# transferia/transferia

Measured on AMD Instinct MI355X. Metric: ChangeItems/sec through CSV parse -> mask(ClientIP)+filter(EventDate) -> devnull, ClickBench hits, HBM-resident input (the PCIe-inclusive rate is `pcie_inclusive`), higher is better.
Workload: dtype u8; 1 GPU; ClickBench hits-1M CSV parse -> mask(ip)+filter(EventDate) -> devnull (BASELINE.json configs[1]); columns=105, parallelism=row-range shard x1, no collective, rows_per_pass=1048576, csv_bytes_per_pass=838371857

## Files before the change

transferia_amd/csrc/tf_common.hpp:

```cpp
#pragma once
#include <hip/hip_runtime.h>

#include <cstdint>
#include <cstdio>
#include <cstring>
#include <memory>
#include <mutex>
#include <unordered_map>
#include <stdexcept>
#include <string>
#include <vector>

#include "../../include/tfgpu.h"

#ifndef TF_DYNAMIC_LDS
#define TF_DYNAMIC_LDS(type, name) extern __shared__ type name[]
#endif

#ifndef TF_GLOBAL_PTR
#define TF_GLOBAL_PTR(T, p) ((T *)(__attribute__((address_space(1))) T *)(p))
#endif

#ifndef TF_CONST_PTR
#define TF_CONST_PTR(T, p) ((const __attribute__((address_space(4))) T *)(p))
#endif

#ifndef TF_KEEP
#define TF_KEEP(x) asm volatile("" ::"v"(x))
#endif
#ifndef TF_OPAQUE
#define TF_OPAQUE(x) asm volatile("" : "+v"(x))
#endif

struct tfgpu_dbatch;

namespace tf {

struct Error : std::runtime_error {
  int code;
  Error(int c, const std::string &m) : std::runtime_error(m), code(c) {}
};
void set_last_error(const std::string &m);
int fail(int code, const std::string &m);

#define TF_HIP(expr)                                                                              \
  do {                                                                                            \
    hipError_t e__ = (expr);                                                                      \
    if (e__ != hipSuccess)                                                                        \
      throw ::tf::Error(TFGPU_ERR_DEVICE, std::string(#expr) + ": " + hipGetErrorString(e__));    \
  } while (0)

struct ProfEntry {
  std::string name;
  int64_t launches = 0;
  double total_ms = 0;
  int64_t units = 0;
};

struct BlockCache {
  std::mutex mu;
  std::unordered_map<size_t, std::vector<void *>> free_;
  size_t cached = 0;
  void *get(size_t cls);
  void put(void *p, size_t cls);
  void trim();
};

struct Context {
  int device = -1;
  hipStream_t stream = nullptr;
  hipStream_t copy_stream = nullptr;
  BlockCache blocks;
  void *pin_base = nullptr;
  size_t pin_cap = 0, pin_off = 0;
  void *pin(size_t bytes);
  template <class T> T *pin_n(size_t n) { return reinterpret_cast<T *>(pin(n * sizeof(T))); }
  bool prof_on = false;
  std::vector<ProfEntry> prof;
  struct Pending { int idx; hipEvent_t a, b; int64_t units = 0; };
  std::vector<Pending> pending;
  std::vector<hipEvent_t> free_events;
  hipEvent_t dense_event = nullptr;
  std::mutex mu;
  int num_cus = 256;
  std::shared_ptr<struct DevMem> pow10tab;
  struct ConstEntry { uint64_t hash; std::vector<uint8_t> bytes; std::shared_ptr<struct DevMem> mem; uint64_t stamp; };
  std::vector<ConstEntry> consts;
  uint64_t const_clock = 0;
  double csv_hint_bpl = 0.0;
  int csv_hint_ncols = -1;

  hipEvent_t get_event();
  void prof_begin(const char *name, Pending &p);
  void prof_end(Pending &p);
  void prof_flush();
};
Context &ctx();
int bind_lane(int lane);
int current_lane();
int lane_device(int lane);
struct LaneScope {
  int prev;
  explicit LaneScope(int lane) : prev(bind_lane(lane)) {}
// ... 37 lines not shown
void sync();

inline bool repr_is_var(int r) { return r == TFGPU_R_STRING || r == TFGPU_R_BYTES || r == TFGPU_R_JSONNUM || r == TFGPU_R_JSON; }
inline size_t repr_width(int r) {
  switch (r) {
    case TFGPU_R_INT8: case TFGPU_R_UINT8: case TFGPU_R_BOOL: return 1;
    case TFGPU_R_INT16: case TFGPU_R_UINT16: return 2;
    case TFGPU_R_INT32: case TFGPU_R_UINT32: case TFGPU_R_FLOAT32: return 4;
    case TFGPU_R_INT64: case TFGPU_R_UINT64: case TFGPU_R_FLOAT64: case TFGPU_R_TIME: case TFGPU_R_DURATION: return 8;
    default: return 0;
  }
}

struct TextView {
  Buf src;
  Buf fstart;
  uint8_t quote = '"';
  bool jsonnum = false;
  bool has_special = true;
  Buf packed;
};
struct DColumn {
  std::string name;
  int dtype = TFGPU_T_INVALID;
  int repr = TFGPU_R_INVALID;
  Buf values, offsets, data, nanos, validity;
  Buf absent;
  uint64_t data_len = 0;
  std::shared_ptr<TextView> view;
  const Buf &payload() const { return (!data && view) ? view->packed : data; }
  bool lazy() const { return !data && view && !view->packed; }
};
void materialize(const struct ::tfgpu_dbatch &b, const std::vector<const DColumn *> *only = nullptr);
void dense(const struct ::tfgpu_dbatch *b, bool absent_ok = false);
void dense_locked(const struct ::tfgpu_dbatch &b);
int lanes_created();
uint64_t lane_generation();
std::unique_ptr<struct ::tfgpu_dbatch> snapshot(const struct ::tfgpu_dbatch &b);
bool has_absent(const struct ::tfgpu_dbatch &b);
Buf validity_minus_absent(const Buf &validity, const Buf &absent, int64_t nrows);
Buf find_device_block(const void *p);
void register_device_block(const Buf &b);

}

namespace tf {
struct PendingRows {
  std::shared_ptr<const struct ::tfgpu_dbatch> src;
  Buf sel;
};
}

struct tfgpu_dbatch {
  int64_t nrows = 0;
  std::vector<tf::DColumn> cols;
  std::shared_ptr<tf::PendingRows> pending;
  void *dense_done = nullptr;
  int dense_lane = -1;
  uint64_t dense_gen = 0;
  std::vector<tf::DColumn> replaced;
  std::vector<std::pair<std::string, int>> schema;
  std::vector<std::string> key_names;
  std::vector<tf::DColumn> old_keys;
  tf::Buf old_present;
  std::string ns, table;
  tf::Buf kind, src_row, part_id;
  tf::Buf col_order;
};

struct tfgpu_dbuf {
  tf::Buf mem;
  uint64_t size = 0;
};

namespace tf {
inline std::unique_ptr<tfgpu_dbatch> shallow_copy(const tfgpu_dbatch &in) { return std::make_unique<tfgpu_dbatch>(in); }
template <class F> void materialize_where(const tfgpu_dbatch &b, F pred) {
  std::vector<const DColumn *> need;
  for (auto &c : b.cols) if (pred(c)) need.push_back(&c);
  materialize(b, &need);
}
void exclusive_scan_u32(const uint32_t *in, uint32_t *out, int64_t n, bool with_total);
void exclusive_scan_u32_segments(uint32_t *inout, int64_t seg_len, int nseg, int64_t seg_stride);
const uint32_t *any_nonzero_to_host(const uint32_t *v, int64_t n);
const uint32_t *segment_totals_to_host(const uint32_t *scanned, int64_t seg_len, int nseg, int64_t seg_stride);
void sum_u32_segments_u64(const uint32_t *in, int64_t seg_len, int nseg, int64_t seg_stride, unsigned long long *totals);

}
```

transferia_amd/csrc/tf_csv.hip:

```cpp
#include <algorithm>
#include <cmath>
#include <cstdio>
#include <type_traits>

#include "tf_devfmt.hpp"
#include "tf_devparse.hpp"
#include "tf_devfloat.hpp"
#include "tf_segcopy.hpp"
#include "tf_textview.hpp"
#include "tf_wave.hpp"
#include "tf_swar.hpp"
#include "tf_gotime.hpp"
#include "tf_f64range.hpp"
#include "tf_plan.hpp"
#include "tf_strictcell.hpp"

#ifdef TF_CSV_ABLATE_BUILD
#define CSV_ABL(x) ((x).ablate)
#else
#define CSV_ABL(x) 0
#endif
namespace tf {

std::unique_ptr<tfgpu_dbatch> compact_rows(const tfgpu_dbatch &in, Buf keep);

static constexpr int NL_THREADS = 256;
#ifndef TF_NL_ITERS
#define TF_NL_ITERS 7
#endif
static constexpr int NL_ITERS = TF_NL_ITERS;
static constexpr int NL_TILE = NL_THREADS * 16 * NL_ITERS;
static constexpr int CSV_GRAN = 64 * 16;
static constexpr int NL_GPT = NL_TILE / CSV_GRAN;
static_assert(NL_TILE == NL_GPT * CSV_GRAN && NL_THREADS * 16 == 4 * CSV_GRAN, "a wave iteration is a granule");

__device__ __forceinline__ uint32_t nl_mask16(uint4 v) {
  uint32_t m = 0;
  const uint32_t w[4] = {v.x, v.y, v.z, v.w};
#pragma unroll
  for (int k = 0; k < 4; k++) {
    uint32_t x = w[k] ^ 0x0A0A0A0Au;
    uint32_t b0 = ((x & 0xFFu) == 0), b1 = ((x & 0xFF00u) == 0), b2 = ((x & 0xFF0000u) == 0), b3 = ((x & 0xFF000000u) == 0);
    m |= (b0 | b1 << 1 | b2 << 2 | b3 << 3) << (4 * k);
  }
  return m;
}
__device__ __forceinline__ uint32_t nl_count16(uint4 v) {
  const uint32_t w[4] = {v.x, v.y, v.z, v.w};
  uint32_t acc = 0;
#pragma unroll
  for (int k = 0; k < 4; k++) {
    const uint32_t x = w[k] ^ 0x0A0A0A0Au;
    const uint32_t z = ~(((x & 0x7F7F7F7Fu) + 0x7F7F7F7Fu) | x) & 0x80808080u;
    acc = __builtin_amdgcn_udot4(z >> 7, 0x01010101u, acc, false);
  }
  return acc;
}

__device__ __forceinline__ uint4 load16_guard(const uint8_t *base, uint64_t pos, uint64_t len) {
  uint4 v = *reinterpret_cast<const uint4 *>(base + pos);
  if (pos + 16 > len) {
    uint32_t w[4] = {v.x, v.y, v.z, v.w};
    for (int i = 0; i < 16; i++) if (pos + i >= len) w[i >> 2] &= ~(0xFFu << (8 * (i & 3)));
    v = make_uint4(w[0], w[1], w[2], w[3]);
  }
  return v;
}

__global__ void __launch_bounds__(NL_THREADS) csv_count_newlines(const uint8_t *__restrict__ data, uint64_t len, uint32_t *__restrict__ gran_counts, int64_t ngran) {
  const uint64_t tile = (uint64_t)blockIdx.x * NL_TILE;
  const int lane = threadIdx.x & 63, wv = threadIdx.x >> 6;
#pragma unroll
  for (int it = 0; it < NL_ITERS; it++) {
    const uint64_t pos = tile + ((uint64_t)it * NL_THREADS + threadIdx.x) * 16;
    uint32_t cnt = 0;
    if (pos < len) cnt = nl_count16(load16_guard(data, pos, len));
    const uint32_t inc = wave_scan_add(cnt);
    const int64_t g = (int64_t)blockIdx.x * NL_GPT + it * 4 + wv;
    if (lane == 63 && g < ngran) gran_counts[g] = inc;
  }
}

__global__ void __launch_bounds__(NL_THREADS) csv_line_index(const uint8_t *__restrict__ data, uint64_t len, const uint32_t *__restrict__ tile_base,
                                                            uint32_t *__restrict__ row_start ) {
  __shared__ uint32_t wsum[NL_THREADS / 64];
  uint64_t tile = (uint64_t)blockIdx.x * NL_TILE;
  uint32_t base = tile_base[(int64_t)blockIdx.x * NL_GPT];
  const int lane = threadIdx.x & 63, wv = threadIdx.x >> 6;
  for (int it = 0; it < NL_ITERS; it++) {
    uint64_t pos = tile + ((uint64_t)it * NL_THREADS + threadIdx.x) * 16;
    uint32_t m = pos < len ? nl_mask16(load16_guard(data, pos, len)) : 0;
    uint32_t c = __popc(m), inc = c;
    for (int d = 1; d < 64; d <<= 1) { uint32_t t = __shfl_up(inc, d, 64); if (lane >= d) inc += t; }
    if (lane == 63) wsum[wv] = inc;
    __syncthreads();
    uint32_t wbase = 0, tot = 0;
    for (int i = 0; i < NL_THREADS / 64; i++) { uint32_t s = wsum[i]; if (i < wv) wbase += s; tot += s; }
    __syncthreads();
    uint32_t k = base + wbase + inc - c;
    while (m) { int b = __ffs(m) - 1; m &= m - 1; row_start[++k] = (uint32_t)(pos + b + 1); }
    base += tot;
  }
}


template <class F> __device__ __forceinline__ uint32_t space_prefix(const F &f, uint32_t i, uint32_t end) {
  uint32_t c = f[i];
  if (c == ' ' || (c >= 9 && c <= 13)) return 1;
  if (c < 0xC2) return 0;
  uint32_t r = end - i;
  if (c == 0xC2 && r >= 2) { uint32_t d = f[i + 1]; return (d == 0x85 || d == 0xA0) ? 2 : 0; }
  if (r >= 3 && (c == 0xE1 || c == 0xE2 || c == 0xE3)) {
    uint32_t d = f[i + 1], e = f[i + 2];
    if (c == 0xE1) return (d == 0x9A && e == 0x80) ? 3 : 0;
    if (c == 0xE3) return (d == 0x80 && e == 0x80) ? 3 : 0;
    if (d == 0x80 && ((e >= 0x80 && e <= 0x8A) || e == 0xA8 || e == 0xA9 || e == 0xAF)) return 3;
    if (d == 0x81 && e == 0x9F) return 3;
  }
  return 0;
}
template <class F> __device__ __forceinline__ uint32_t space_suffix(const F &f, uint32_t a, uint32_t b) {
  uint32_t c = f[b - 1];
  if (c == ' ' || (c >= 9 && c <= 13)) return 1;
  if (c < 0x80) return 0;
  if (b - a >= 2 && f[b - 2] == 0xC2 && (c == 0x85 || c == 0xA0)) return 2;
  if (b - a >= 3 && space_prefix(f, b - 3, b) == 3) return 3;
  return 0;
}

struct CsvOpts {
  uint8_t delim, quote, escape, double_quote, include_missing, strings_can_be_null, quoted_strings_can_be_null, pad;
  int32_t n_null, n_true, n_false;
  const uint32_t *list_off;
  const uint8_t *list_data;
  GtSet user_tp;
  GtSet cast_tp;
  const uint8_t *dp;
  uint32_t dp_len;
  uint32_t multiline;
  const uint64_t *p128;
};

__device__ __forceinline__ bool any_quote(const uint32_t *qmask, uint32_t lo, uint32_t hi) {
  if (lo >= hi) return false;
  const uint32_t w0 = lo >> 5, w1 = (hi - 1) >> 5;
  for (uint32_t w = w0; w <= w1; w++) {
    uint32_t m = qmask[w];
    if (w == w0) m &= ~0u << (lo & 31);
    if (w == w1) m &= ~0u >> (31 - ((hi - 1) & 31));
    if (m) return true;
  }
  return false;
}

// ... 2258 lines not shown
```

transferia_amd/csrc/tf_mask.hip:

```cpp
#include "tf_plan.hpp"
#include "tf_rows.hpp"
#include "tf_devrow.hpp"
#include "tf_emit.hpp"

namespace tf {
__constant__ uint32_t SHA_K[64] = {
    0x428a2f98, 0x71374491, 0xb5c0fbcf, 0xe9b5dba5, 0x3956c25b, 0x59f111f1, 0x923f82a4, 0xab1c5ed5, 0xd807aa98, 0x12835b01, 0x243185be,
    0x550c7dc3, 0x72be5d74, 0x80deb1fe, 0x9bdc06a7, 0xc19bf174, 0xe49b69c1, 0xefbe4786, 0x0fc19dc6, 0x240ca1cc, 0x2de92c6f, 0x4a7484aa,
    0x5cb0a9dc, 0x76f988da, 0x983e5152, 0xa831c66d, 0xb00327c8, 0xbf597fc7, 0xc6e00bf3, 0xd5a79147, 0x06ca6351, 0x14292967, 0x27b70a85,
    0x2e1b2138, 0x4d2c6dfc, 0x53380d13, 0x650a7354, 0x766a0abb, 0x81c2c92e, 0x92722c85, 0xa2bfe8a1, 0xa81a664b, 0xc24b8b70, 0xc76c51a3,
    0xd192e819, 0xd6990624, 0xf40e3585, 0x106aa070, 0x19a4c116, 0x1e376c08, 0x2748774c, 0x34b0bcb5, 0x391c0cb3, 0x4ed8aa4a, 0x5b9cca4f,
    0x682e6ff3, 0x748f82ee, 0x78a5636f, 0x84c87814, 0x8cc70208, 0x90befffa, 0xa4506ceb, 0xbef9a3f7, 0xc67178f2};

__device__ __forceinline__ uint32_t rotr32(uint32_t x, int n) { return __builtin_rotateright32(x, n); }

__device__ __forceinline__ void sha256_compress(uint32_t st[8], uint32_t w[16]) {
  uint32_t a = st[0], b = st[1], c = st[2], d = st[3], e = st[4], f = st[5], g = st[6], h = st[7];
#pragma unroll
  for (int i = 0; i < 64; i++) {
    if (i >= 16) {
      uint32_t w15 = w[(i - 15) & 15], w2 = w[(i - 2) & 15];
      uint32_t s0 = rotr32(w15, 7) ^ rotr32(w15, 18) ^ (w15 >> 3);
      uint32_t s1 = rotr32(w2, 17) ^ rotr32(w2, 19) ^ (w2 >> 10);
      w[i & 15] = w[i & 15] + s0 + w[(i - 7) & 15] + s1;
    }
    uint32_t t1 = h + (rotr32(e, 6) ^ rotr32(e, 11) ^ rotr32(e, 25)) + ((e & f) ^ (~e & g)) + SHA_K[i] + w[i & 15];
    uint32_t t2 = (rotr32(a, 2) ^ rotr32(a, 13) ^ rotr32(a, 22)) + ((a & b) ^ (a & c) ^ (b & c));
    h = g; g = f; f = e; e = d + t1; d = c; c = b; b = a; a = t1 + t2;
  }
  st[0] += a; st[1] += b; st[2] += c; st[3] += d; st[4] += e; st[5] += f; st[6] += g; st[7] += h;
}

struct MaskParams {
  DCol col;
  uint32_t ipad[8], opad[8];
  int64_t nrows;
  uint8_t *out;
  const int32_t *sel;
};

struct Text24 {
  uint64_t t0 = 0, t1 = 0, t2 = 0; uint32_t n = 0;
  __device__ __forceinline__ void put_word(uint64_t w, uint32_t k) {
    const uint32_t at = n & 7u, sh = at * 8, seg = n >> 3;
    const uint64_t lo = w << sh, hi = (w >> 1) >> (63 - sh);
    if (seg == 0) { t0 |= lo; t1 |= hi; } else if (seg == 1) { t1 |= lo; t2 |= hi; } else t2 |= lo;
    n += k;
  }
  __device__ __forceinline__ void put(uint32_t c) { put_word(c & 0xFFu, 1); }
};
__device__ __forceinline__ bool mask_small_int(const DCol &c, int64_t r, Text24 &s) {
  if (!is_valid(c, r)) { s.put_word(0x3E6C696E3Cull , 5); return true; }
  switch (c.repr) {
    case TFGPU_R_INT8: emit_i64(s, ((const int8_t *)c.values)[r]); return true;
    case TFGPU_R_INT16: emit_i64(s, ((const int16_t *)c.values)[r]); return true;
    case TFGPU_R_INT32: emit_i64(s, ((const int32_t *)c.values)[r]); return true;
    case TFGPU_R_INT64: emit_i64(s, ((const int64_t *)c.values)[r]); return true;
    case TFGPU_R_UINT8: emit_u64(s, ((const uint8_t *)c.values)[r]); return true;
    case TFGPU_R_UINT16: emit_u64(s, ((const uint16_t *)c.values)[r]); return true;
    case TFGPU_R_UINT32: emit_u64(s, ((const uint32_t *)c.values)[r]); return true;
    case TFGPU_R_UINT64: emit_u64(s, ((const uint64_t *)c.values)[r]); return true;
    default: return false;
  }
}

__global__ void __launch_bounds__(256) mask_hmac_kernel(MaskParams p) {
  const int64_t ro = (int64_t)blockIdx.x * blockDim.x + threadIdx.x;
  if (ro >= p.nrows) return;
  const int64_t r = p.sel ? (int64_t)p.sel[ro] : ro;
  uint32_t st[8], w[16];
#pragma unroll
  for (int i = 0; i < 8; i++) st[i] = p.ipad[i];
  const bool small_int = p.col.repr >= TFGPU_R_INT8 && p.col.repr <= TFGPU_R_UINT64;
  if (small_int) {
    Text24 s;
    mask_small_int(p.col, r, s);
    const uint32_t len = s.n;
    s.put_word(0x80, 1);
    w[0] = __builtin_bswap32((uint32_t)s.t0); w[1] = __builtin_bswap32((uint32_t)(s.t0 >> 32));
    w[2] = __builtin_bswap32((uint32_t)s.t1); w[3] = __builtin_bswap32((uint32_t)(s.t1 >> 32));
    w[4] = __builtin_bswap32((uint32_t)s.t2); w[5] = __builtin_bswap32((uint32_t)(s.t2 >> 32));
#pragma unroll
    for (int i = 6; i < 15; i++) w[i] = 0;
    w[15] = (64 + len) * 8;
    sha256_compress(st, w);
  } else {
  uint8_t buf[64];
  const uint8_t *ext;
  int len = serialize_small(p.col, r, buf, &ext);
  int off = 0;
  uint64_t bits = (uint64_t)(64 + len) * 8;
  bool pad_done = false, len_done = false;
  while (!len_done) {
#pragma unroll
    for (int i = 0; i < 16; i++) w[i] = 0;
    int take = len - off; if (take > 64) take = 64; if (take < 0) take = 0;
    for (int i = 0; i < take; i++) {
      uint32_t b = ext ? ext[off + i] : buf[off + i];
      w[i >> 2] |= b << (24 - 8 * (i & 3));
    }
    off += take;
    if (take < 64 && !pad_done) { w[take >> 2] |= 0x80u << (24 - 8 * (take & 3)); pad_done = true; if (take < 56) { w[14] = (uint32_t)(bits >> 32); w[15] = (uint32_t)bits; len_done = true; } }
    else if (pad_done) { w[14] = (uint32_t)(bits >> 32); w[15] = (uint32_t)bits; len_done = true; }
    sha256_compress(st, w);
  }
  }
#pragma unroll
  for (int i = 0; i < 8; i++) w[i] = st[i];
  w[8] = 0x80000000u;
#pragma unroll
  for (int i = 9; i < 15; i++) w[i] = 0;
  w[15] = (64 + 32) * 8;
  uint32_t so[8];
#pragma unroll
  for (int i = 0; i < 8; i++) so[i] = p.opad[i];
  sha256_compress(so, w);
  uint4 *dst = reinterpret_cast<uint4 *>(p.out + ro * 64);
#pragma unroll
  for (int q = 0; q < 4; q++) {
    uint32_t o[4];
#pragma unroll
    for (int k = 0; k < 4; k++) {
      uint32_t word = so[q * 2 + (k >> 1)];
      uint32_t half = (k & 1) ? (word & 0xFFFF) : (word >> 16);
      uint32_t n0 = (half >> 12) & 15, n1 = (half >> 8) & 15, n2 = (half >> 4) & 15, n3 = half & 15;
      auto hx = [](uint32_t n) { return n + (n < 10 ? '0' : 'a' - 10); };
      o[k] = hx(n0) | hx(n1) << 8 | hx(n2) << 16 | hx(n3) << 24;
    }
    dst[q] = make_uint4(o[0], o[1], o[2], o[3]);
  }
}

__global__ void fill_offsets_stride_kernel(uint32_t *off, int64_t n, uint32_t stride) {
  int64_t i = (int64_t)blockIdx.x * blockDim.x + threadIdx.x;
  if (i <= n) off[i] = (uint32_t)(i * stride);
}


void mask_precheck(const tfgpu_plan &p, const tfgpu_dbatch &in) {
  for (auto &c : (in.pending ? in.pending->src->cols : in.cols)) {
    if (!p.mask_has(c.name)) continue;
    bool done = false;
    for (auto &r : in.replaced) if (r.name == c.name) done = true;
    if (done) continue;
    require_serializable(c, "mask_field");
    if ((uint64_t)in.nrows * 64 > 0xFFFFFFFFull) throw Error(TFGPU_ERR_UNSUPPORTED, "mask_field: batch too large for 32-bit offsets; split the batch by rows");
  }
}

std::unique_ptr<tfgpu_dbatch> apply_mask(const tfgpu_plan &p, const tfgpu_dbatch &in) {
  auto out = shallow_copy(in);
  for (auto &sc : out->schema) if (p.mask_has(sc.first)) sc.second = TFGPU_T_UTF8;
  hipStream_t st = ctx().stream;
  const tfgpu_dbatch &from = in.pending ? *in.pending->src : in;
  const int32_t *sel = in.pending ? ptr<int32_t>(in.pending->sel) : nullptr;
  auto replaced_at = [&](const std::string &name) -> int { for (size_t i = 0; i < in.replaced.size(); i++) if (in.replaced[i].name == name) return (int)i; return -1; };
  materialize_where(from, [&](const DColumn &c) { return p.mask_has(c.name) && replaced_at(c.name) < 0; });
  const int64_t n = in.nrows;
  auto mask_one = [&](const DColumn &c, const int32_t *through) {
    require_serializable(c, "mask_field");
    if ((uint64_t)n * 64 > 0xFFFFFFFFull) throw Error(TFGPU_ERR_UNSUPPORTED, "mask_field: batch too large for 32-bit offsets; split the batch by rows");
    DColumn o;
    o.name = c.name; o.dtype = TFGPU_T_UTF8; o.repr = TFGPU_R_STRING;
    o.data_len = (uint64_t)n * 64;
    o.data = dalloc(o.data_len);
    o.offsets = dalloc((size_t)(n + 1) * 4);
    MaskParams mp;
    mp.col = dcol_of(c);
    std::memcpy(mp.ipad, p.ipad_state, sizeof mp.ipad);
    std::memcpy(mp.opad, p.opad_state, sizeof mp.opad);
    mp.nrows = n; mp.out = ptr<uint8_t>(o.data); mp.sel = through;
    {
      KernelTimer t("mask_hmac_sha256", n);
      if (n) mask_hmac_kernel<<<grid_for(n, 256), 256, 0, st>>>(mp);
    }
    fill_offsets_stride_kernel<<<grid_for(n + 1, 256), 256, 0, st>>>(ptr<uint32_t>(o.offsets), n, 64);
    return o;
  };
  if (!in.pending) {
    for (auto &c : out->cols) if (p.mask_has(c.name)) {
      const Buf ab = c.absent;
      c = mask_one(c, nullptr);
      if (ab) { c.absent = ab; c.validity = validity_minus_absent(nullptr, ab, n); }
    }
    return out;
  }
  for (auto &c : from.cols) {
    if (!p.mask_has(c.name)) continue;
    const int ri = replaced_at(c.name);
    if (ri >= 0) out->replaced[(size_t)ri] = mask_one(in.replaced[(size_t)ri], nullptr);
    else out->replaced.push_back(mask_one(c, sel));
  }
  return out;
}
}
```

transferia_amd/csrc/tf_rows.hip:

```cpp
#include <chrono>
#include <thread>

#include "tf_rows.hpp"
#include "tf_devrow.hpp"
#include "tf_segcopy.hpp"
#include "tf_textview.hpp"

namespace tf {
__global__ void __launch_bounds__(256) build_selection_kernel(const uint32_t *__restrict__ keep_scan, int64_t n, int32_t *__restrict__ sel) {
  int64_t i = (int64_t)blockIdx.x * blockDim.x + threadIdx.x;
  if (i >= n) return;
  uint32_t a = keep_scan[i], b = keep_scan[i + 1];
  if (a != b) sel[a] = (int32_t)i;
}

struct GFix { const void *in; void *out; int32_t width; int32_t pad; };
template <class T> __device__ __forceinline__ void gather_run(const GFix *__restrict__ a, int lo, int hi, int32_t s, int64_t k) {
  constexpr int U = 8;
  int i = lo;
  for (; i + U <= hi; i += U) {
    T v[U];
#pragma unroll
    for (int q = 0; q < U; q++) v[q] = TF_GLOBAL_PTR(const T, a[i + q].in)[s];
#pragma unroll
// ... 109 lines not shown
    o.name = c.name; o.dtype = c.dtype; o.repr = c.repr;
    if (repr_is_var(c.repr)) {
      size_t si = vr.size();
      o.offsets = subbuf(lens_all, si * (size_t)seg_stride * 4, (size_t)(m + 1) * 4);
      if (!c.lazy() || eager_text) o.data = dalloc(c.data_len + 8);
      o.data_len = c.data_len;
      if (c.lazy() && !eager_text) {
        if (!c.view->src) throw Error(TFGPU_ERR_INVALID, "internal: text column " + c.name + " lost its source text");
        auto v = std::make_shared<TextView>();
        v->src = c.view->src; v->fstart = dalloc((size_t)std::max<int64_t>(m, 1) * 4);
        v->has_special = c.view->has_special; v->quote = c.view->quote; v->jsonnum = c.view->jsonnum;
        fx.push_back(GFix{c.view->fstart->p, v->fstart->p, 4, 0});
        o.view = std::move(v);
        o.data = nullptr;
        vr.push_back(GVar{ptr<uint32_t>(c.offsets), nullptr, ptr<uint32_t>(o.offsets), nullptr, nullptr, 0, 0, 0});
      } else if (c.lazy()) {
        if (!c.view->src) throw Error(TFGPU_ERR_INVALID, "internal: text column " + c.name + " lost its source text");
        vr.push_back(GVar{ptr<uint32_t>(c.offsets), ptr<uint8_t>(c.view->src), ptr<uint32_t>(o.offsets), ptr<uint8_t>(o.data), ptr<uint32_t>(c.view->fstart), c.view->quote, c.view->jsonnum ? 1u : 0u, c.view->has_special ? 1u : 0u});
      } else vr.push_back(GVar{ptr<uint32_t>(c.offsets), ptr<uint8_t>(c.payload()), ptr<uint32_t>(o.offsets), ptr<uint8_t>(o.data), nullptr, 0, 0, 0});
      var_cols.push_back(ai);
    } else {
      size_t w = repr_width(c.repr);
      o.values = dalloc((size_t)m * w);
      fx.push_back(GFix{c.values->p, o.values->p, (int32_t)w, 0});
      if (c.nanos) { o.nanos = dalloc((size_t)m * 4); fx.push_back(GFix{c.nanos->p, o.nanos->p, 4, 0}); }
    }
    if (c.validity) { o.validity = dalloc((size_t)(m + 7) / 8 + 1); bits.push_back(GBit{ptr<uint8_t>(c.validity), ptr<uint8_t>(o.validity)}); }
    if (c.absent) { o.absent = dalloc((size_t)(m + 7) / 8 + 1); bits.push_back(GBit{ptr<uint8_t>(c.absent), ptr<uint8_t>(o.absent)}); }
    (ai < ncur ? out->cols : out->old_keys).push_back(std::move(o));
  }
  auto out_at = [&](size_t i) -> DColumn & { return i < ncur ? out->cols[i] : out->old_keys[i - ncur]; };
  if (in.old_present) { out->old_present = dalloc((size_t)(m + 7) / 8 + 1); bits.push_back(GBit{ptr<uint8_t>(in.old_present), ptr<uint8_t>(out->old_present)}); }
  if (in.kind) { out->kind = dalloc((size_t)m); fx.push_back(GFix{in.kind->p, out->kind->p, 1, 0}); }
  if (in.part_id) { out->part_id = dalloc((size_t)m * 4); fx.push_back(GFix{in.part_id->p, out->part_id->p, 4, 0}); }
  out->src_row = dalloc((size_t)m * 4);
  if (in.src_row) fx.push_back(GFix{in.src_row->p, out->src_row->p, 4, 0});
  uint32_t *const ident = in.src_row ? nullptr : ptr<uint32_t>(out->src_row);

  if (m && !bits.empty()) {
    Buf bb = upload_const(bits.data(), bits.size() * sizeof(GBit));
    gather_bitmap_all<<<dim3(grid_for((m + 7) / 8, 256), (unsigned)bits.size()), 256, 0, st>>>(ptr<GBit>(bb), sp, m);
  }
  std::stable_sort(fx.begin(), fx.end(), [](const GFix &x, const GFix &y) { return x.width < y.width; });
  int nw[4] = {0, 0, 0, 0};
  for (auto &x : fx) nw[x.width == 1 ? 0 : x.width == 2 ? 1 : x.width == 4 ? 2 : 3]++;
  const int nfx[4] = {nw[0], nw[1], nw[2], nw[3]};
  if (fx.empty()) fx.push_back(GFix{nullptr, nullptr, 0, 0});
  Buf bfx = upload_const(fx.data(), fx.size() * sizeof(GFix));
  if (m) gather_fixed_all<<<g, 256, 0, st>>>(ptr<GFix>(bfx), nfx[0], nfx[1], nfx[2], nfx[3], ident, sp, m);
  if (nvar) {
    Buf bvr = upload_const(vr.data(), vr.size() * sizeof(GVar));
    if (m) gather_len_all<<<g, 256, 0, st>>>(ptr<GVar>(bvr), nvar, sp, m);
    exclusive_scan_u32_segments(ptr<uint32_t>(lens_all), m, nvar, seg_stride);
    if (m) {
      std::vector<GVar> lng, sht;
      for (size_t i = 0; i < vr.size(); i++) if (vr[i].out_data) ((col_at(var_cols[i]).data_len >= (uint64_t)in.nrows * 8) ? lng : sht).push_back(vr[i]);
      Buf blng = upload_const(lng.data(), lng.size() * sizeof(GVar)), bsht = upload_const(sht.data(), sht.size() * sizeof(GVar));
      if (!lng.empty()) gather_bytes_all<1><<<dim3(grid_for(m, 256), (unsigned)lng.size()), 256, 0, st>>>(ptr<GVar>(blng), sp, m);
      if (!sht.empty()) gather_bytes_cells<<<dim3(grid_for(m, 256), (unsigned)sht.size()), 256, 0, st>>>(ptr<GVar>(bsht), sp, m);
      std::vector<GVar> lz;
      for (auto &x : vr) if (x.fstart && x.has_special) lz.push_back(x);
      if (!lz.empty()) {
        Buf blz = upload_const(lz.data(), lz.size() * sizeof(GVar));
        gather_text_special<<<dim3(grid_for(m, 256), (unsigned)lz.size()), 256, 0, st>>>(ptr<GVar>(blz), sp, m);
      }
    }
    Buf tot = dalloc((size_t)nvar * 4);
    collect_totals<<<1, 64, 0, st>>>(ptr<uint32_t>(lens_all), seg_stride, m, nvar, ptr<uint32_t>(tot));
    const uint32_t *h = d2h_u32(tot->p, (size_t)nvar);
    sync();
    for (int i = 0; i < nvar; i++) out_at(var_cols[(size_t)i]).data_len = h[i];
  }
  return out;
}

std::unique_ptr<tfgpu_dbatch> gather_rows(const tfgpu_dbatch &in, const Buf &sel, int64_t m) { return gather_batch(in, sel, m); }

static bool lazy_rows_on() {
  static const bool off = [] { const char *e = std::getenv("TFGPU_LAZY_ROWS"); return e && e[0] == '0'; }();
  return !off;
}
std::unique_ptr<tfgpu_dbatch> compact(const tfgpu_dbatch &in, Buf keep , bool lazy) {
  int64_t n = in.nrows;
  exclusive_scan_u32(ptr<uint32_t>(keep), ptr<uint32_t>(keep), n, true);
  const uint32_t *hm = d2h_u32(ptr<uint32_t>(keep) + n);
  Buf sel = dalloc((size_t)n * 4 + 4);
  if (n) build_selection_kernel<<<grid_for(n, 256), 256, 0, ctx().stream>>>(ptr<uint32_t>(keep), n, ptr<int32_t>(sel));
  sync();
  const uint32_t m = *hm;
  if ((int64_t)m == n) return shallow_copy(in);
  if (lazy && lazy_rows_on() && !in.pending && m) {
    auto out = std::make_unique<tfgpu_dbatch>();
    out->nrows = m; out->ns = in.ns; out->table = in.table; out->schema = in.schema; out->key_names = in.key_names;
    auto pr = std::make_shared<PendingRows>();
    pr->src = std::make_shared<const tfgpu_dbatch>(in);
    pr->sel = sel;
    out->pending = std::move(pr);
    return out;
  }
  return gather_batch(in, sel, m);
}

static std::mutex g_dense_mu;
static void dense_hold() {
  static const int ms = [] { const char *e = std::getenv("TFGPU_DENSE_HOLD_MS"); return e ? std::atoi(e) : 0; }();
  if (ms > 0) std::this_thread::sleep_for(std::chrono::milliseconds(ms));
}
static void wait_dense_nolock(const tfgpu_dbatch &b) {
  if (b.dense_done && b.dense_lane != current_lane() && b.dense_gen == lane_generation()) TF_HIP(hipStreamWaitEvent(ctx().stream, (hipEvent_t)b.dense_done, 0));
}
std::unique_ptr<tfgpu_dbatch> snapshot(const tfgpu_dbatch &b) {
  std::unique_ptr<tfgpu_dbatch> c;
  { std::lock_guard<std::mutex> dl(g_dense_mu); c = std::make_unique<tfgpu_dbatch>(b); }
  if (c->pending) dense_hold();
  return c;
}
void dense_locked(const tfgpu_dbatch &b) {
  std::lock_guard<std::mutex> dl(g_dense_mu);
  if (!b.pending) { wait_dense_nolock(b); return; }
  tfgpu_dbatch &mb = const_cast<tfgpu_dbatch &>(b);
  std::shared_ptr<PendingRows> pr = b.pending;
  std::unique_ptr<tfgpu_dbatch> g = gather_batch(*pr->src, pr->sel, b.nrows, b.replaced.empty() ? nullptr : &b.replaced);
  mb.cols = std::move(g->cols); mb.old_keys = std::move(g->old_keys); mb.old_present = g->old_present;
  mb.kind = g->kind; mb.src_row = g->src_row; mb.part_id = g->part_id;
  mb.replaced.clear();
  if (lanes_created() > 1) {
    Context &cx = ctx();
    if (!cx.dense_event) TF_HIP(hipEventCreateWithFlags(&cx.dense_event, hipEventDisableTiming));
    TF_HIP(hipEventRecord(cx.dense_event, cx.stream));
    mb.dense_done = (void *)cx.dense_event;
    mb.dense_lane = current_lane();
    mb.dense_gen = lane_generation();
  }
  mb.pending.reset();
}
bool has_absent(const tfgpu_dbatch &b) {
  std::lock_guard<std::mutex> dl(g_dense_mu);
  if (b.col_order) return true;
  for (auto &c : (b.pending ? b.pending->src->cols : b.cols)) if (c.absent) return true;
  return false;
}
void wait_dense(const tfgpu_dbatch &b) { std::lock_guard<std::mutex> dl(g_dense_mu); wait_dense_nolock(b); }
void refuse_absent(const tfgpu_dbatch &b) {
  if (has_absent(b))
    throw Error(TFGPU_ERR_UNSUPPORTED, "the batch holds ABSENT cells (rows whose ColumnNames leave a column out: TOASTed updates, tfgpu_column.absent); this entry computes on values and "
                                       "does not read them — tfgpu_collapse, tfgpu_keys_changed, tfgpu_partition, view / download do");
}
void dense(const tfgpu_dbatch *b, bool absent_ok) {
  if (!b) return;
  if (!absent_ok) refuse_absent(*b);
  { std::lock_guard<std::mutex> dl(g_dense_mu); if (!b->pending) { wait_dense_nolock(*b); return; } }
  dense_hold();
  std::lock_guard<std::mutex> lk(ctx().mu);
  dense_locked(*b);
}

std::unique_ptr<tfgpu_dbatch> compact_rows(const tfgpu_dbatch &in, Buf keep) { return compact(in, keep); }

__global__ void part_keep_kernel(const uint32_t *part_id, int64_t n, uint32_t d, uint32_t *keep) {
  int64_t r = (int64_t)blockIdx.x * blockDim.x + threadIdx.x;
  if (r < n) keep[r] = part_id[r] == d ? 1u : 0u;
}
__global__ void part_scatter_kernel(const uint32_t *keep_scan, int64_t n, uint32_t base, int32_t *sel) {
  int64_t i = (int64_t)blockIdx.x * blockDim.x + threadIdx.x;
  if (i >= n) return;
  const uint32_t a = keep_scan[i], b = keep_scan[i + 1];
  if (a != b) sel[base + a] = (int32_t)i;
}
std::unique_ptr<tfgpu_dbatch> partition_rows(const tfgpu_dbatch &in, int nparts, int64_t *counts) {
  if (!in.part_id) throw Error(TFGPU_ERR_INVALID, "tfgpu_partition: the batch has no part_id (apply sharder_transformer first)");
// ... 20 lines not shown
```

transferia_amd/csrc/tf_scan.hip:

```cpp
#include "tf_common.hpp"

namespace tf {

static constexpr int SCAN_THREADS = 256;
static constexpr int SCAN_ITEMS = 16;
static constexpr int SCAN_TILE = SCAN_THREADS * SCAN_ITEMS;
static constexpr int64_t RAW_SUMS_MAX = 1024;

__device__ __forceinline__ uint32_t wave_incl_scan(uint32_t v) {
  const int lane = threadIdx.x & 63;
#pragma unroll
  for (int d = 1; d < 64; d <<= 1) {
    uint32_t t = __shfl_up(v, d, 64);
    if (lane >= d) v += t;
  }
  return v;
}

__device__ __forceinline__ uint32_t block_excl_scan(uint32_t v, uint32_t *total, uint32_t *lds ) {
  const int lane = threadIdx.x & 63, w = threadIdx.x >> 6;
  uint32_t inc = wave_incl_scan(v);
  if (lane == 63) lds[w] = inc;
  __syncthreads();
  uint32_t base = 0, tot = 0;
#pragma unroll
  for (int i = 0; i < SCAN_THREADS / 64; i++) { uint32_t s = lds[i]; if (i < w) base += s; tot += s; }
  __syncthreads();
  *total = tot;
  return base + inc - v;
}

__global__ void __launch_bounds__(SCAN_THREADS) scan_reduce_kernel(const uint32_t *__restrict__ in, uint32_t *__restrict__ sums,
                                                                  int64_t n, int64_t seg_stride, int64_t nblocks) {
  __shared__ uint32_t lds[4];
  const uint32_t *src = in + (int64_t)blockIdx.y * seg_stride;
  int64_t base = (int64_t)blockIdx.x * SCAN_TILE + (int64_t)threadIdx.x * SCAN_ITEMS;
  uint32_t s = 0;
  if (base + SCAN_ITEMS <= n && ((reinterpret_cast<uintptr_t>(src + base) & 15) == 0)) {
    const uint4 *p = reinterpret_cast<const uint4 *>(src + base);
#pragma unroll
    for (int i = 0; i < SCAN_ITEMS / 4; i++) { uint4 v = p[i]; s += v.x + v.y + v.z + v.w; }
  } else {
    for (int i = 0; i < SCAN_ITEMS; i++) if (base + i < n) s += src[base + i];
  }
  uint32_t tot;
  block_excl_scan(s, &tot, lds);
  if (threadIdx.x == 0) sums[(int64_t)blockIdx.y * nblocks + blockIdx.x] = tot;
}

__global__ void __launch_bounds__(SCAN_THREADS) scan_apply_kernel(const uint32_t *__restrict__ in, uint32_t *__restrict__ out,
                                                                 const uint32_t *__restrict__ block_base, int64_t n,
                                                                 int64_t seg_stride, int64_t nblocks, int write_total, int raw_sums) {
  __shared__ uint32_t lds[4];
  uint32_t bb = 0;
  if (block_base) {
    const uint32_t *bs = block_base + (int64_t)blockIdx.y * nblocks;
    if (raw_sums) {
      uint32_t part = 0;
      for (int64_t i = threadIdx.x; i < (int64_t)blockIdx.x; i += SCAN_THREADS) part += bs[i];
      block_excl_scan(part, &bb, lds);
    } else bb = bs[blockIdx.x];
  }
  const uint32_t *src = in + (int64_t)blockIdx.y * seg_stride;
  uint32_t *dst = out + (int64_t)blockIdx.y * seg_stride;
  int64_t base = (int64_t)blockIdx.x * SCAN_TILE + (int64_t)threadIdx.x * SCAN_ITEMS;
  uint32_t v[SCAN_ITEMS];
  bool fast = base + SCAN_ITEMS <= n && ((reinterpret_cast<uintptr_t>(src + base) & 15) == 0);
  if (fast) {
    const uint4 *p = reinterpret_cast<const uint4 *>(src + base);
#pragma unroll
    for (int i = 0; i < SCAN_ITEMS / 4; i++) { uint4 q = p[i]; v[4 * i] = q.x; v[4 * i + 1] = q.y; v[4 * i + 2] = q.z; v[4 * i + 3] = q.w; }
  } else {
#pragma unroll
    for (int i = 0; i < SCAN_ITEMS; i++) v[i] = (base + i < n) ? src[base + i] : 0;
  }
  uint32_t s = 0;
#pragma unroll
  for (int i = 0; i < SCAN_ITEMS; i++) s += v[i];
  uint32_t tot;
  uint32_t ex = block_excl_scan(s, &tot, lds) + bb;
#pragma unroll
  for (int i = 0; i < SCAN_ITEMS; i++) { uint32_t t = v[i]; v[i] = ex; ex += t; }
  if (fast) {
    uint4 *p = reinterpret_cast<uint4 *>(dst + base);
#pragma unroll
    for (int i = 0; i < SCAN_ITEMS / 4; i++) p[i] = make_uint4(v[4 * i], v[4 * i + 1], v[4 * i + 2], v[4 * i + 3]);
  } else {
#pragma unroll
    for (int i = 0; i < SCAN_ITEMS; i++) if (base + i < n) dst[base + i] = v[i];
  }
  if (write_total && base <= n - 1 && n - 1 < base + SCAN_ITEMS) dst[n] = ex;
}

static void scan_impl(const uint32_t *in, uint32_t *out, int64_t n, int64_t seg_stride, int nseg, bool with_total) {
  if (n <= 0) {
    if (with_total) for (int s = 0; s < nseg; s++) TF_HIP(hipMemsetAsync(out + (int64_t)s * seg_stride, 0, 4, ctx().stream));
    return;
  }
  hipStream_t st = ctx().stream;
  int64_t nblocks = (n + SCAN_TILE - 1) / SCAN_TILE;
  dim3 grid((unsigned)nblocks, (unsigned)nseg);
  if (nblocks == 1) {
    scan_apply_kernel<<<grid, SCAN_THREADS, 0, st>>>(in, out, nullptr, n, seg_stride, 1, with_total ? 1 : 0, 0);
    return;
  }
  Buf sums = dalloc((size_t)nblocks * nseg * 4 + 4);
  scan_reduce_kernel<<<grid, SCAN_THREADS, 0, st>>>(in, ptr<uint32_t>(sums), n, seg_stride, nblocks);
  const bool raw = nblocks <= RAW_SUMS_MAX;
  if (!raw) scan_impl(ptr<uint32_t>(sums), ptr<uint32_t>(sums), nblocks, nblocks, nseg, false);
  scan_apply_kernel<<<grid, SCAN_THREADS, 0, st>>>(in, out, ptr<uint32_t>(sums), n, seg_stride, nblocks, with_total ? 1 : 0, raw ? 1 : 0);
}

__global__ void __launch_bounds__(SCAN_THREADS) sum_u64_kernel(const uint32_t *__restrict__ in, int64_t n, int64_t seg_stride, unsigned long long *totals) {
  const uint32_t *src = in + (int64_t)blockIdx.y * seg_stride;
  unsigned long long s = 0;
  for (int64_t i = (int64_t)blockIdx.x * SCAN_THREADS + threadIdx.x; i < n; i += (int64_t)gridDim.x * SCAN_THREADS) s += src[i];
  for (int d = 32; d; d >>= 1) s += __shfl_down(s, d, 64);
  if ((threadIdx.x & 63) == 0 && s) atomicAdd(totals + blockIdx.y, s);
}

void sum_u32_segments_u64(const uint32_t *in, int64_t seg_len, int nseg, int64_t seg_stride, unsigned long long *totals) {
  if (nseg <= 0 || seg_len <= 0) return;
  const int64_t nb = std::min<int64_t>((seg_len + SCAN_THREADS * 8 - 1) / (SCAN_THREADS * 8), 1024);
  sum_u64_kernel<<<dim3((unsigned)nb, (unsigned)nseg), SCAN_THREADS, 0, ctx().stream>>>(in, seg_len, seg_stride, totals);
}

__global__ void segment_totals_kernel(const uint32_t *lens_all, int64_t seg_stride, int64_t n, int nseg, uint32_t *out) {
  for (int t = threadIdx.x; t < nseg; t += blockDim.x) out[t] = lens_all[(int64_t)t * seg_stride + n];
}
const uint32_t *segment_totals_to_host(const uint32_t *scanned, int64_t seg_len, int nseg, int64_t seg_stride) {
  if (nseg <= 0) return nullptr;
  Buf out = dalloc((size_t)nseg * 4);
  segment_totals_kernel<<<1, 256, 0, ctx().stream>>>(scanned, seg_stride, seg_len, nseg, ptr<uint32_t>(out));
  return d2h_u32(out->p, (size_t)nseg);
}

__global__ void __launch_bounds__(256) any_nonzero_kernel(const uint32_t *v, int64_t n, uint32_t *flag) {
  bool hit = false;
  for (int64_t i = (int64_t)blockIdx.x * 256 + threadIdx.x; i < n; i += (int64_t)gridDim.x * 256) hit |= v[i] != 0;
  if (__ballot(hit) && (threadIdx.x & 63) == 0) atomicOr(flag, 1u);
}
const uint32_t *any_nonzero_to_host(const uint32_t *v, int64_t n) {
  Buf flag = dalloc_zero(4);
  if (n > 0) any_nonzero_kernel<<<(unsigned)std::min<int64_t>((n + 255) / 256, 1024), 256, 0, ctx().stream>>>(v, n, ptr<uint32_t>(flag));
  return d2h_u32(flag->p, 1);
}

void exclusive_scan_u32(const uint32_t *in, uint32_t *out, int64_t n, bool with_total) {
  KernelTimer t("scan_u32");
  scan_impl(in, out, n, 0, 1, with_total);
}

void exclusive_scan_u32_segments(uint32_t *inout, int64_t seg_len, int nseg, int64_t seg_stride) {
  if (nseg <= 0) return;
  KernelTimer t("scan_u32_segments");
  scan_impl(inout, inout, seg_len, seg_stride, nseg, true);
}

}
```

Measured before the change: 910.0 million rows/s.

## Fuse compaction scan with selection, fold offsets fill into mask, stream newline loads

```diff
diff --git a/transferia_amd/csrc/tf_common.hpp b/transferia_amd/csrc/tf_common.hpp
--- a/transferia_amd/csrc/tf_common.hpp
+++ b/transferia_amd/csrc/tf_common.hpp
@@ -19,6 +19,15 @@
 
 #ifndef TF_GLOBAL_PTR
 #define TF_GLOBAL_PTR(T, p) ((T *)(__attribute__((address_space(1))) T *)(p))
+#endif
+
+#ifndef TF_LOAD16_STREAM
+__device__ __forceinline__ uint4 tf_load16_stream(const void *p) {
+  typedef uint32_t v4u __attribute__((ext_vector_type(4)));
+  const v4u t = __builtin_nontemporal_load(reinterpret_cast<const v4u *>(p));
+  return make_uint4(t[0], t[1], t[2], t[3]);
+}
+#define TF_LOAD16_STREAM(p) tf_load16_stream(p)
 #endif
 
 #ifndef TF_CONST_PTR
@@ -222,6 +231,7 @@
 }
 void exclusive_scan_u32(const uint32_t *in, uint32_t *out, int64_t n, bool with_total);
 void exclusive_scan_u32_segments(uint32_t *inout, int64_t seg_len, int nseg, int64_t seg_stride);
+bool select_kept_u32(const uint32_t *keep, int64_t n, int32_t *sel, uint32_t *count);
 const uint32_t *any_nonzero_to_host(const uint32_t *v, int64_t n);
 const uint32_t *segment_totals_to_host(const uint32_t *scanned, int64_t seg_len, int nseg, int64_t seg_stride);
 void sum_u32_segments_u64(const uint32_t *in, int64_t seg_len, int nseg, int64_t seg_stride, unsigned long long *totals);
diff --git a/transferia_amd/csrc/tf_csv.hip b/transferia_amd/csrc/tf_csv.hip
--- a/transferia_amd/csrc/tf_csv.hip
+++ b/transferia_amd/csrc/tf_csv.hip
@@ -70,6 +70,17 @@
 __global__ void __launch_bounds__(NL_THREADS) csv_count_newlines(const uint8_t *__restrict__ data, uint64_t len, uint32_t *__restrict__ gran_counts, int64_t ngran) {
   const uint64_t tile = (uint64_t)blockIdx.x * NL_TILE;
   const int lane = threadIdx.x & 63, wv = threadIdx.x >> 6;
+  if (tile + NL_TILE <= len) {
+    uint4 v[NL_ITERS];
+#pragma unroll
+    for (int it = 0; it < NL_ITERS; it++) v[it] = TF_LOAD16_STREAM(data + tile + ((uint64_t)it * NL_THREADS + threadIdx.x) * 16);
+#pragma unroll
+    for (int it = 0; it < NL_ITERS; it++) {
+      const uint32_t inc = wave_scan_add(nl_count16(v[it]));
+      if (lane == 63) gran_counts[(int64_t)blockIdx.x * NL_GPT + it * 4 + wv] = inc;
+    }
+    return;
+  }
 #pragma unroll
   for (int it = 0; it < NL_ITERS; it++) {
     const uint64_t pos = tile + ((uint64_t)it * NL_THREADS + threadIdx.x) * 16;
diff --git a/transferia_amd/csrc/tf_mask.hip b/transferia_amd/csrc/tf_mask.hip
--- a/transferia_amd/csrc/tf_mask.hip
+++ b/transferia_amd/csrc/tf_mask.hip
@@ -36,6 +36,7 @@
   uint32_t ipad[8], opad[8];
   int64_t nrows;
   uint8_t *out;
+  uint32_t *offsets;
   const int32_t *sel;
 };
 
@@ -129,11 +130,8 @@
     }
     dst[q] = make_uint4(o[0], o[1], o[2], o[3]);
   }
-}
-
-__global__ void fill_offsets_stride_kernel(uint32_t *off, int64_t n, uint32_t stride) {
-  int64_t i = (int64_t)blockIdx.x * blockDim.x + threadIdx.x;
-  if (i <= n) off[i] = (uint32_t)(i * stride);
+  p.offsets[ro] = (uint32_t)(ro * 64);
+  if (ro == p.nrows - 1) p.offsets[p.nrows] = (uint32_t)(p.nrows * 64);
 }
 
 
@@ -169,12 +167,12 @@
     mp.col = dcol_of(c);
     std::memcpy(mp.ipad, p.ipad_state, sizeof mp.ipad);
     std::memcpy(mp.opad, p.opad_state, sizeof mp.opad);
-    mp.nrows = n; mp.out = ptr<uint8_t>(o.data); mp.sel = through;
+    mp.nrows = n; mp.out = ptr<uint8_t>(o.data); mp.offsets = ptr<uint32_t>(o.offsets); mp.sel = through;
     {
       KernelTimer t("mask_hmac_sha256", n);
       if (n) mask_hmac_kernel<<<grid_for(n, 256), 256, 0, st>>>(mp);
     }
-    fill_offsets_stride_kernel<<<grid_for(n + 1, 256), 256, 0, st>>>(ptr<uint32_t>(o.offsets), n, 64);
+    if (!n) TF_HIP(hipMemsetAsync(o.offsets->p, 0, 4, st));
     return o;
   };
   if (!in.pending) {
diff --git a/transferia_amd/csrc/tf_rows.hip b/transferia_amd/csrc/tf_rows.hip
--- a/transferia_amd/csrc/tf_rows.hip
+++ b/transferia_amd/csrc/tf_rows.hip
@@ -215,10 +215,14 @@
 }
 std::unique_ptr<tfgpu_dbatch> compact(const tfgpu_dbatch &in, Buf keep , bool lazy) {
   int64_t n = in.nrows;
-  exclusive_scan_u32(ptr<uint32_t>(keep), ptr<uint32_t>(keep), n, true);
-  const uint32_t *hm = d2h_u32(ptr<uint32_t>(keep) + n);
   Buf sel = dalloc((size_t)n * 4 + 4);
-  if (n) build_selection_kernel<<<grid_for(n, 256), 256, 0, ctx().stream>>>(ptr<uint32_t>(keep), n, ptr<int32_t>(sel));
+  const uint32_t *hm;
+  if (select_kept_u32(ptr<uint32_t>(keep), n, ptr<int32_t>(sel), ptr<uint32_t>(keep) + n)) hm = d2h_u32(ptr<uint32_t>(keep) + n);
+  else {
+    exclusive_scan_u32(ptr<uint32_t>(keep), ptr<uint32_t>(keep), n, true);
+    hm = d2h_u32(ptr<uint32_t>(keep) + n);
+    if (n) build_selection_kernel<<<grid_for(n, 256), 256, 0, ctx().stream>>>(ptr<uint32_t>(keep), n, ptr<int32_t>(sel));
+  }
   sync();
   const uint32_t m = *hm;
   if ((int64_t)m == n) return shallow_copy(in);
diff --git a/transferia_amd/csrc/tf_scan.hip b/transferia_amd/csrc/tf_scan.hip
--- a/transferia_amd/csrc/tf_scan.hip
+++ b/transferia_amd/csrc/tf_scan.hip
@@ -1,71 +1,15 @@
 #include "tf_common.hpp"
+#include "tf_wave.hpp"
 
 namespace tf {
 
 static constexpr int SCAN_THREADS = 256;
+static constexpr int SCAN_WAVES = SCAN_THREADS / 64;
 static constexpr int SCAN_ITEMS = 16;
 static constexpr int SCAN_TILE = SCAN_THREADS * SCAN_ITEMS;
 static constexpr int64_t RAW_SUMS_MAX = 1024;
 
-__device__ __forceinline__ uint32_t wave_incl_scan(uint32_t v) {
-  const int lane = threadIdx.x & 63;
-#pragma unroll
-  for (int d = 1; d < 64; d <<= 1) {
-    uint32_t t = __shfl_up(v, d, 64);
-    if (lane >= d) v += t;
-  }
-  return v;
-}
-
-__device__ __forceinline__ uint32_t block_excl_scan(uint32_t v, uint32_t *total, uint32_t *lds ) {
-  const int lane = threadIdx.x & 63, w = threadIdx.x >> 6;
-  uint32_t inc = wave_incl_scan(v);
-  if (lane == 63) lds[w] = inc;
-  __syncthreads();
-  uint32_t base = 0, tot = 0;
-#pragma unroll
-  for (int i = 0; i < SCAN_THREADS / 64; i++) { uint32_t s = lds[i]; if (i < w) base += s; tot += s; }
-  __syncthreads();
-  *total = tot;
-  return base + inc - v;
-}
-
-__global__ void __launch_bounds__(SCAN_THREADS) scan_reduce_kernel(const uint32_t *__restrict__ in, uint32_t *__restrict__ sums,
-                                                                  int64_t n, int64_t seg_stride, int64_t nblocks) {
-  __shared__ uint32_t lds[4];
-  const uint32_t *src = in + (int64_t)blockIdx.y * seg_stride;
-  int64_t base = (int64_t)blockIdx.x * SCAN_TILE + (int64_t)threadIdx.x * SCAN_ITEMS;
-  uint32_t s = 0;
-  if (base + SCAN_ITEMS <= n && ((reinterpret_cast<uintptr_t>(src + base) & 15) == 0)) {
-    const uint4 *p = reinterpret_cast<const uint4 *>(src + base);
-#pragma unroll
-    for (int i = 0; i < SCAN_ITEMS / 4; i++) { uint4 v = p[i]; s += v.x + v.y + v.z + v.w; }
-  } else {
-    for (int i = 0; i < SCAN_ITEMS; i++) if (base + i < n) s += src[base + i];
-  }
-  uint32_t tot;
-  block_excl_scan(s, &tot, lds);
-  if (threadIdx.x == 0) sums[(int64_t)blockIdx.y * nblocks + blockIdx.x] = tot;
-}
-
-__global__ void __launch_bounds__(SCAN_THREADS) scan_apply_kernel(const uint32_t *__restrict__ in, uint32_t *__restrict__ out,
-                                                                 const uint32_t *__restrict__ block_base, int64_t n,
-                                                                 int64_t seg_stride, int64_t nblocks, int write_total, int raw_sums) {
-  __shared__ uint32_t lds[4];
-  uint32_t bb = 0;
-  if (block_base) {
-    const uint32_t *bs = block_base + (int64_t)blockIdx.y * nblocks;
-    if (raw_sums) {
-      uint32_t part = 0;
-      for (int64_t i = threadIdx.x; i < (int64_t)blockIdx.x; i += SCAN_THREADS) part += bs[i];
-      block_excl_scan(part, &bb, lds);
-    } else bb = bs[blockIdx.x];
-  }
-  const uint32_t *src = in + (int64_t)blockIdx.y * seg_stride;
-  uint32_t *dst = out + (int64_t)blockIdx.y * seg_stride;
-  int64_t base = (int64_t)blockIdx.x * SCAN_TILE + (int64_t)threadIdx.x * SCAN_ITEMS;
-  uint32_t v[SCAN_ITEMS];
-  bool fast = base + SCAN_ITEMS <= n && ((reinterpret_cast<uintptr_t>(src + base) & 15) == 0);
+__device__ __forceinline__ void scan_load16(const uint32_t *__restrict__ src, int64_t base, int64_t n, bool fast, uint32_t v[SCAN_ITEMS]) {
   if (fast) {
     const uint4 *p = reinterpret_cast<const uint4 *>(src + base);
 #pragma unroll
@@ -74,11 +18,64 @@
 #pragma unroll
     for (int i = 0; i < SCAN_ITEMS; i++) v[i] = (base + i < n) ? src[base + i] : 0;
   }
+}
+
+__global__ void __launch_bounds__(SCAN_THREADS) scan_reduce_kernel(const uint32_t *__restrict__ in, uint32_t *__restrict__ sums,
+                                                                  int64_t n, int64_t seg_stride, int64_t nblocks) {
+  __shared__ uint32_t lds[SCAN_WAVES];
+  const uint32_t *src = in + (int64_t)blockIdx.y * seg_stride;
+  const int lane = threadIdx.x & 63, w = threadIdx.x >> 6;
+  const int64_t base = (int64_t)blockIdx.x * SCAN_TILE + (int64_t)threadIdx.x * SCAN_ITEMS;
+  uint32_t v[SCAN_ITEMS];
+  scan_load16(src, base, n, base + SCAN_ITEMS <= n && ((reinterpret_cast<uintptr_t>(src + base) & 15) == 0), v);
   uint32_t s = 0;
 #pragma unroll
   for (int i = 0; i < SCAN_ITEMS; i++) s += v[i];
-  uint32_t tot;
-  uint32_t ex = block_excl_scan(s, &tot, lds) + bb;
+  s = wave_scan_add(s);
+  if (lane == 63) lds[w] = s;
+  __syncthreads();
+  if (threadIdx.x == 0) {
+    uint32_t tot = 0;
+#pragma unroll
+    for (int i = 0; i < SCAN_WAVES; i++) tot += lds[i];
+    sums[(int64_t)blockIdx.y * nblocks + blockIdx.x] = tot;
+  }
+}
+
+template <bool SELECT>
+__global__ void __launch_bounds__(SCAN_THREADS) scan_apply_kernel(const uint32_t *__restrict__ in, uint32_t *__restrict__ out,
+                                                                 const uint32_t *__restrict__ block_base, int64_t n,
+                                                                 int64_t seg_stride, int64_t nblocks, int write_total, int raw_sums, uint32_t *__restrict__ count) {
+  __shared__ uint32_t lds[2][SCAN_WAVES];
+  const int lane = threadIdx.x & 63, w = threadIdx.x >> 6;
+  const uint32_t *src = in + (int64_t)blockIdx.y * seg_stride;
+  uint32_t *dst = out + (int64_t)blockIdx.y * seg_stride;
+  const int64_t base = (int64_t)blockIdx.x * SCAN_TILE + (int64_t)threadIdx.x * SCAN_ITEMS;
+  uint32_t v[SCAN_ITEMS];
+  const bool fast = base + SCAN_ITEMS <= n && ((reinterpret_cast<uintptr_t>(src + base) & 15) == 0);
+  scan_load16(src, base, n, fast, v);
+  uint32_t part = 0;
+  if (block_base) {
+    const uint32_t *bs = block_base + (int64_t)blockIdx.y * nblocks;
+    if (raw_sums) { for (int64_t i = threadIdx.x; i < (int64_t)blockIdx.x; i += SCAN_THREADS) part += bs[i]; }
+    else if (threadIdx.x == 0) part = bs[blockIdx.x];
+  }
+  uint32_t s = 0;
+#pragma unroll
+  for (int i = 0; i < SCAN_ITEMS; i++) s += v[i];
+  const uint32_t inc = wave_scan_add(s);
+  part = wave_scan_add(part);
+  if (lane == 63) { lds[0][w] = inc; lds[1][w] = part; }
+  __syncthreads();
+  uint32_t ex = inc - s;
+#pragma unroll
+  for (int i = 0; i < SCAN_WAVES; i++) { ex += lds[1][i]; if (i < w) ex += lds[0][i]; }
+  if (SELECT) {
+#pragma unroll
+    for (int i = 0; i < SCAN_ITEMS; i++) { const uint32_t t = v[i]; if (t) out[ex] = (uint32_t)(base + i); ex += t; }
+    if (base <= n - 1 && n - 1 < base + SCAN_ITEMS) *count = ex;
+    return;
+  }
 #pragma unroll
   for (int i = 0; i < SCAN_ITEMS; i++) { uint32_t t = v[i]; v[i] = ex; ex += t; }
   if (fast) {
@@ -101,14 +98,28 @@
   int64_t nblocks = (n + SCAN_TILE - 1) / SCAN_TILE;
   dim3 grid((unsigned)nblocks, (unsigned)nseg);
   if (nblocks == 1) {
-    scan_apply_kernel<<<grid, SCAN_THREADS, 0, st>>>(in, out, nullptr, n, seg_stride, 1, with_total ? 1 : 0, 0);
+    scan_apply_kernel<false><<<grid, SCAN_THREADS, 0, st>>>(in, out, nullptr, n, seg_stride, 1, with_total ? 1 : 0, 0, nullptr);
     return;
   }
   Buf sums = dalloc((size_t)nblocks * nseg * 4 + 4);
   scan_reduce_kernel<<<grid, SCAN_THREADS, 0, st>>>(in, ptr<uint32_t>(sums), n, seg_stride, nblocks);
   const bool raw = nblocks <= RAW_SUMS_MAX;
   if (!raw) scan_impl(ptr<uint32_t>(sums), ptr<uint32_t>(sums), nblocks, nblocks, nseg, false);
-  scan_apply_kernel<<<grid, SCAN_THREADS, 0, st>>>(in, out, ptr<uint32_t>(sums), n, seg_stride, nblocks, with_total ? 1 : 0, raw ? 1 : 0);
+  scan_apply_kernel<false><<<grid, SCAN_THREADS, 0, st>>>(in, out, ptr<uint32_t>(sums), n, seg_stride, nblocks, with_total ? 1 : 0, raw ? 1 : 0, nullptr);
+}
+
+bool select_kept_u32(const uint32_t *keep, int64_t n, int32_t *sel, uint32_t *count) {
+  const int64_t nblocks = (n + SCAN_TILE - 1) / SCAN_TILE;
+  if (n <= 0 || nblocks > RAW_SUMS_MAX) return false;
+  KernelTimer t("scan_u32");
+  hipStream_t st = ctx().stream;
+  Buf sums;
+  if (nblocks > 1) {
+    sums = dalloc((size_t)nblocks * 4 + 4);
+    scan_reduce_kernel<<<(unsigned)nblocks, SCAN_THREADS, 0, st>>>(keep, ptr<uint32_t>(sums), n, 0, nblocks);
+  }
+  scan_apply_kernel<true><<<(unsigned)nblocks, SCAN_THREADS, 0, st>>>(keep, reinterpret_cast<uint32_t *>(sel), ptr<uint32_t>(sums), n, 0, nblocks, 0, 1, count);
+  return true;
 }
 
 __global__ void __launch_bounds__(SCAN_THREADS) sum_u64_kernel(const uint32_t *__restrict__ in, int64_t n, int64_t seg_stride, unsigned long long *totals) {
```

Measured after the change: 959.4 million rows/s (median of 6 runs). 5.4% higher.
